# swift-nav/albatross

Measured on AMD Instinct MI355X. Metric: GP fits/sec (Gram+Chol+solve) at N=16384 fp64, higher is better.
Workload: dtype f64

## Files before the change

### albatross_amd/csrc/api.hip

```cpp
#include <algorithm>
#include <atomic>
#include <cmath>
#include <cstring>
#include <chrono>
#include <cstdio>
#include <new>
#include <thread>

#include "api_internal.h"
#include <deque>
#include <mutex>
#include <tuple>
#include <unordered_map>
#include "trace.h"
#include "pub.h"

namespace agp {

void DeviceFeatures::release() {
  for (void *&p : owned) {
    if (p) (void)hipFree(p);
    p = nullptr;
  }
  v = FeatView{};
// ... 136 lines not shown
  return n;
}

static constexpr long long BACKSUB_COOP_MAX_N = 2047;
static agp_context::Tuning read_tuning() {
  agp_context::Tuning t;
  auto flag = [](const char *name, bool dflt) {
    const char *e = getenv(name);
    return e && e[0] ? e[0] == '1' : dflt;
  };
  auto number = [](const char *name, long long dflt) {
    const char *e = getenv(name);
    return e && e[0] ? atoll(e) : dflt;
  };
  t.panel_fused = flag("AGP_PANEL_FUSED", true);
  t.step_below = number("AGP_STEP_BELOW", 4608);
  t.gram_sop = flag("AGP_GRAM_SOP", true);
  t.backsub_coop = flag("AGP_BACKSUB_COOP", true);
  t.backsub_coop_max = number("AGP_BACKSUB_COOP_MAX", BACKSUB_COOP_MAX_N);
  t.mixed_bf16 = flag("AGP_MIXED_BF16", true);
  t.mixed_f16 = flag("AGP_MIXED_F16", true);
  set_f16x2_kernel((int)number("AGP_F16X2_LDS_PAD", 8192), (int)number("AGP_F16X2_TERMS", 4), (int)number("AGP_F16X2_CHUNK", 32));
  t.mixed_nbo = number("AGP_MIXED_NBO", 512);
  t.fp64_nbo = number("AGP_FP64_NBO", 0);
  if (t.fp64_nbo <= 512 || t.fp64_nbo % 128 != 0) t.fp64_nbo = 0;
  set_bf16x3_kernel((int)number("AGP_BF16X3_KERNEL", 2), (int)number("AGP_BF16X3_LDS_PAD", 8192));
  t.sparse_pivoted = flag("AGP_SPARSE_PIVOTED", false);
  t.predict_chunk = number("AGP_PREDICT_CHUNK", 0);
  t.shard_block = number("AGP_SHARD_BLOCK", 0);
  t.shard_force_comm = flag("AGP_SHARD_FORCE_COMM", false);
  t.shard_host_pacing = flag("AGP_SHARD_HOST_PACING", false);
  if (const char *e = getenv("AGP_SHARD_MASK_GFLOP")) t.shard_mask_gflop = atof(e);
  t.merge_above = number("AGP_MERGE_ABOVE", 8704);
  return t;
}

int agp_context_create(int device_id, agp_context **out) {
  if (!out) return AGP_ERR_INVALID_ARGUMENT;
  *out = nullptr;
  int n = 0;
  if (hipGetDeviceCount(&n) != hipSuccess || n <= 0) return AGP_ERR_NO_DEVICE;
  if (device_id < 0 || device_id >= n) return AGP_ERR_INVALID_ARGUMENT;
  agp_context_impl *ctx = new (std::nothrow) agp_context_impl();
  if (!ctx) return AGP_ERR_INVALID_ARGUMENT;
  ctx->device = device_id;
  ctx->tune = read_tuning();
  agp::g_gram_sop = ctx->tune.gram_sop;
  AGP_HIP_CHECK(ctx, hipSetDevice(device_id));
  {
    int lo = 0, hi = 0;
    AGP_HIP_CHECK(ctx, hipDeviceGetStreamPriorityRange(&lo, &hi));
    AGP_HIP_CHECK(ctx, hipStreamCreateWithPriority(&ctx->stream, hipStreamNonBlocking, hi));
    AGP_HIP_CHECK(ctx, hipStreamCreateWithPriority(&ctx->stream2, hipStreamNonBlocking, lo));
    AGP_HIP_CHECK(ctx, hipStreamCreateWithPriority(&ctx->stream3, hipStreamNonBlocking, lo));
    AGP_HIP_CHECK(ctx, hipEventCreateWithFlags(&ctx->ev_inv, hipEventDisableTiming));
    AGP_HIP_CHECK(ctx, hipEventCreateWithFlags(&ctx->ev_c, hipEventDisableTiming));
    int cus = 256;
    (void)hipDeviceGetAttribute(&cus, hipDeviceAttributeMultiprocessorCount, device_id);
    ctx->cus = cus;
    const int keep = cus / 8 * 7 / 8 * 8;
    if (keep > 0 && keep < cus) {
      uint32_t mask[16] = {0};
      for (int i = 0; i < keep && i < 512; ++i) mask[i / 32] |= 1u << (i % 32);
      if (hipExtStreamCreateWithCUMask(&ctx->stream_masked, (uint32_t)((cus + 31) / 32), mask) != hipSuccess) {
        (void)hipGetLastError();
        ctx->stream_masked = nullptr;
// ... 11 lines not shown
  for (auto &e : ctx->stage_ev) AGP_HIP_CHECK(ctx, hipEventCreate(&e));
  for (auto &sl : ctx->ext.slots) AGP_HIP_CHECK(ctx, hipMalloc(&sl.dev, sizeof(DevProgram)));
  *out = ctx;
  return AGP_OK;
}

void agp_context_destroy(agp_context *c) {
  if (!c) return;
  agp_context_impl *ctx = static_cast<agp_context_impl *>(c);
  (void)hipSetDevice(ctx->device);
  (void)hipDeviceSynchronize();
  for (agp_context *h : ctx->helpers) agp_context_destroy(h);
  ctx->helpers.clear();
  for (auto &sl : ctx->ext.slots)
    if (sl.dev) (void)hipFree(sl.dev);
  for (auto e : ctx->gemm_events) (void)hipEventDestroy(e);
  for (auto e : ctx->stage_ev)
    if (e) (void)hipEventDestroy(e);
  if (ctx->partial_ws) (void)hipFree(ctx->partial_ws);
  if (ctx->ws_A) (void)agp::dev_release(ctx->ws_A);
  if (ctx->pool_A) (void)agp::dev_release(ctx->pool_A);
  if (ctx->pool_K) (void)agp::dev_release(ctx->pool_K);
  if (ctx->ws_refine) (void)hipFree(ctx->ws_refine);
  if (ctx->p32) (void)hipFree(ctx->p32);
  if (ctx->f16_scales) (void)hipFree(ctx->f16_scales);
  if (ctx->pool_L32) (void)hipFree(ctx->pool_L32);
  if (ctx->pool_aux) (void)agp::dev_release(ctx->pool_aux);
  if (ctx->pool_shard) (void)agp::dev_release(ctx->pool_shard);
  if (ctx->pool_sparse) (void)agp::dev_release(ctx->pool_sparse);
  if (ctx->pool_batch) (void)agp::dev_release(ctx->pool_batch);
  if (ctx->ws_aux) (void)hipFree(ctx->ws_aux);
  if (ctx->d_zpub) (void)hipFree(ctx->d_zpub);
  if (ctx->d_dpub) (void)hipFree(ctx->d_dpub);
  if (ctx->shard_flags) (void)hipFree(ctx->shard_flags);
  if (ctx->d_headcnt) (void)hipFree(ctx->d_headcnt);
  if (ctx->h_stage) (void)hipHostFree(ctx->h_stage);
  if (ctx->d_flags) (void)hipFree(ctx->d_flags);
  if (ctx->h_flags) (void)hipHostFree(ctx->h_flags);
  if (ctx->ev_a) (void)hipEventDestroy(ctx->ev_a);
  if (ctx->ev_b) (void)hipEventDestroy(ctx->ev_b);
  if (ctx->stream) (void)hipStreamDestroy(ctx->stream);
  if (ctx->stream2) (void)hipStreamDestroy(ctx->stream2);
  if (ctx->stream3) (void)hipStreamDestroy(ctx->stream3);
  if (ctx->ev_inv) (void)hipEventDestroy(ctx->ev_inv);
  if (ctx->stream_masked) (void)hipStreamDestroy(ctx->stream_masked);
  if (ctx->stream_comm) (void)hipStreamDestroy(ctx->stream_comm);
  if (ctx->ev_c) (void)hipEventDestroy(ctx->ev_c);
  delete ctx;
  agp::dev_cache_trim();
}

int agp_context_synchronize(agp_context *ctx) {
  if (!ctx) return AGP_ERR_INVALID_ARGUMENT;
  AGP_HIP_CHECK(ctx, hipSetDevice(ctx->device));
  AGP_HIP_CHECK(ctx, hipDeviceSynchronize());
  return AGP_OK;
}

int agp_device_malloc(agp_context *ctx, int64_t bytes, void **out) {
  if (!ctx || !out || bytes <= 0) return AGP_ERR_INVALID_ARGUMENT;
  *out = nullptr;
  AGP_HIP_CHECK(ctx, hipSetDevice(ctx->device));
  AGP_HIP_CHECK(ctx, hipMalloc(out, (size_t)bytes));
  return AGP_OK;
}

// ... 1643 lines not shown
```

### albatross_amd/csrc/chol.hip

```cpp
#include <cstdlib>
#include "common.h"
#include "mfma_f64.h"
#include "gemm_tiles.h"
#include "trsm_kernel.h"
#include "pub.h"

namespace agp {
void launch_set_identity_batched(hipStream_t s, double *B, long long ld, long long stride, long long m, long long count);

__device__ __forceinline__ double readlane_f64(double v, int lane) {
  const long long b = __double_as_longlong(v);
  const int lo = __builtin_amdgcn_readlane((int)(b & 0xffffffffll), lane);
  const int hi = __builtin_amdgcn_readlane((int)(b >> 32), lane);
  return __longlong_as_double(((long long)hi << 32) | (unsigned int)lo);
}

__device__ __forceinline__ double rsqrt_nr(double x) {
  double y = __builtin_amdgcn_rsq(x);
  const double h = 0.5 * x;
  y = y * (1.5 - h * y * y);
  y = y * (1.5 - h * y * y);
  return y;
}

struct PotrfArgs {
  double *A;
  long long lda;
  long long k0;
  int nbk;
  double *img;
  double *y;
  int *flags;
  double *scalars;
  long long batch_A = 0, batch_img = 0, batch_y = 0, batch_scalars = 0, batch_flags = 0, batch_zpub = 0;
  double *zpub = nullptr;
  long long below = 0;
  double *dpub = nullptr;
  unsigned trail_first = 0xffffffffu;
  unsigned hold_index = 0xffffffffu, hold_count = 0;
  unsigned long long *rowcnt = nullptr;
  unsigned long long rowcnt_expect = 0;
  long long trail_tiles = 0, trail_workers = 1;
};


template <int J>
__device__ __forceinline__ double bcast_row(double v) {
  double r;
  asm("s_nop 1\n\tv_mov_b64_dpp %0, %1 row_newbcast:%2 row_mask:0xf bank_mask:0xf" : "=v"(r) : "v"(v), "n"(J));
  return r;
}

template <int J>
__device__ __forceinline__ void fnmac_bcast_row(double &acc, double src, double a) {
  asm("s_nop 1\n\tv_fmac_f64_dpp %0, -%1, %2 row_newbcast:%3 row_mask:0xf bank_mask:0xf"
      : "+v"(acc) : "v"(src), "v"(a), "n"(J));
}

__device__ __forceinline__ double vmul(double a, double b) {
  double r;
  asm volatile("v_mul_f64 %0, %1, %2" : "=v"(r) : "v"(a), "v"(b));
  return r;
}
__device__ __forceinline__ double vfma(double a, double b, double c) {
  double r;
  asm volatile("v_fma_f64 %0, %1, %2, %3" : "=v"(r) : "v"(a), "v"(b), "v"(c));
  return r;
}
__device__ __forceinline__ double vfnma(double a, double b, double c) {
  double r;
  asm volatile("v_fma_f64 %0, -%1, %2, %3" : "=v"(r) : "v"(a), "v"(b), "v"(c));
  return r;
}
__device__ __forceinline__ double vrsq(double a) {
  double r;
// ... 168 lines not shown
  double *Adiag = p.A + p.k0 * p.lda + p.k0;
  if constexpr (UPD) {
    double v[NTILE];
    unsigned long long t0 = 0;
    for (int spin = 0;; ++spin) {
      bool ok = true;
#pragma unroll
      for (int t = 0; t < NTILE; ++t) v[t] = load_pub(p.dpub + t * (MB * MB) + tid);
#pragma unroll
      for (int t = 0; t < NTILE; ++t) ok = ok && !is_unpublished(v[t]);
      if (__all(ok)) break;
      if (spin == 0) t0 = __builtin_amdgcn_s_memrealtime();
      else if ((spin & 63) == 0 && poll_expired(t0, p.flags)) break;
      __builtin_amdgcn_s_sleep(2);
    }
#pragma unroll
    for (int t = 0; t < NTILE; ++t) T[t * (MB * MB) + tid] = v[t];
  } else {
    const int r = tid & 15, c = tid >> 4;
    double v[NTILE];
#pragma unroll
    for (int ib = 0; ib < NMB; ++ib)
#pragma unroll
      for (int kb = 0; kb <= ib; ++kb) {
        const int gr = ib * MB + r, gc = kb * MB + c;
        double x;
        if (gr < nbk && gc < nbk) x = (gr >= gc) ? Adiag[gc * p.lda + gr] : 0.;
        else x = (gr == gc) ? 1. : 0.;
        v[ib * (ib + 1) / 2 + kb] = x;
      }
#pragma unroll
    for (int t = 0; t < NTILE; ++t) T[t * (MB * MB) + c * MB + r] = v[t];
  }
  if (tid < NB) ys[tid] = (p.y && tid < nbk) ? p.y[tid] : 0.;
  __syncthreads();

  int bad_pivot = 0;
  if (wave == 0) micro_potrf_inv<PUB>(T + tile_off(0, 0), Wc, p.img + tile_off(0, 0), lane, ln, 0, bad_pivot);
  __syncthreads();
  AGP_PROBE(1);

#pragma unroll 1
  for (int jb = 0; jb < NMB; ++jb) {
    const int o = jb * MB;
    const double *W = Wc + (jb & 1) * (MB * MB);
    for (int ib = jb + 1 + wave; ib < NMB; ib += 4) {
      double *X = T + tile_off(ib, jb);
      v4d acc0 = v4zero(), acc1 = v4zero();
      acc0 = mfma16(W[(0 + lg) * MB + ln], X[(0 + lg) * MB + ln], acc0);
      acc1 = mfma16(W[(4 + lg) * MB + ln], X[(4 + lg) * MB + ln], acc1);
      acc0 = mfma16(W[(8 + lg) * MB + ln], X[(8 + lg) * MB + ln], acc0);
      acc1 = mfma16(W[(12 + lg) * MB + ln], X[(12 + lg) * MB + ln], acc1);
#pragma unroll
      for (int r = 0; r < 4; ++r) {
        const double x = acc0[r] + acc1[r];
        X[(lg + 4 * r) * MB + ln] = x;
        if constexpr (PUB) store_pub(p.img + tile_off(ib, jb) + (lg + 4 * r) * MB + ln, -x);
        else p.img[tile_off(ib, jb) + (lg + 4 * r) * MB + ln] = -x;
      }
    }
    if (wave == 3) {
      double zz = 0.;
#pragma unroll
      for (int c = 0; c < MB; ++c) zz += W[c * MB + ln] * ys[o + c];
      if (lane < MB) ys[o + ln] = zz;
    }
    __syncthreads();
// ... 137 lines not shown
  const double *Xd = p.A + (p.k0 - NB) * p.lda + p.k0;
  const double *Dd = p.A + p.k0 * p.lda + p.k0;
  const int ra = kb * MB + ln, rb = ib * MB + ln;
  const bool oka = ra < p.nbk, okb = rb < p.nbk;
  v4d acc[4] = {v4zero(), v4zero(), v4zero(), v4zero()};
#pragma unroll
  for (int r = 0; r < 4; ++r) {
    const int gr = ib * MB + ln, gc = kb * MB + lg + 4 * r;
    double x;
    if (gr < p.nbk && gc < p.nbk) x = (gr >= gc) ? Dd[gc * p.lda + gr] : 0.;
    else x = (gr == gc) ? 1. : 0.;
    acc[0][r] = x;
  }
  {
    double av[32], bv[32];
#pragma unroll
    for (int s2 = 0; s2 < 32; ++s2) {
      const long long k = 4 * s2 + lg;
      av[s2] = oka ? Xd[k * p.lda + ra] : 0.;
      bv[s2] = okb ? Xd[k * p.lda + rb] : 0.;
    }
#pragma unroll
    for (int s2 = 0; s2 < 32; ++s2) acc[s2 & 3] = mfma16(-av[s2], bv[s2], acc[s2 & 3]);
  }
  const v4d out = (acc[0] + acc[1]) + (acc[2] + acc[3]);
#pragma unroll
  for (int r = 0; r < 4; ++r) {
    const int gr = ib * MB + ln, gc = kb * MB + lg + 4 * r;
    store_pub(p.dpub + tile * (MB * MB) + (lg + 4 * r) * MB + ln, (gr >= gc) ? out[r] : 0.);
  }
}

template <bool UPD>
__device__ __forceinline__ void trsm_fused_body(const PotrfArgs &p, int first_block) {
  const int tid = threadIdx.x, lane = tid & 63, wave = tid >> 6;
  const int ln = lane & 15, lg = lane >> 4;
  const long long n0 = ((long long)(blockIdx.x - first_block) * 4 + wave) * 16;
  const bool active = n0 < p.below;
  const bool nok = active && n0 + ln < p.below;
  double *base = p.A + p.k0 * p.lda + (p.k0 + p.nbk) + (n0 + ln);
  const bool handed = UPD && p.rowcnt != nullptr;
  if (handed) {
    if (tid == 0) {
      const unsigned long long *c = p.rowcnt + (blockIdx.x - first_block);
      const unsigned long long t0 = __builtin_amdgcn_s_memrealtime();
      for (int spin = 1; __hip_atomic_load(c, __ATOMIC_RELAXED, __HIP_MEMORY_SCOPE_AGENT) < p.rowcnt_expect; ++spin) {
        if ((spin & 63) == 0 && poll_expired(t0, p.flags)) break;
        __builtin_amdgcn_s_sleep(8);
      }
      __atomic_thread_fence(__ATOMIC_ACQUIRE);
    }
    __syncthreads();
  }
  if (!active) return;
  v4d Y[NMB];
#pragma unroll
  for (int jb = 0; jb < NMB; ++jb)
#pragma unroll
    for (int r = 0; r < 4; ++r) {
      const int m = jb * MB + lg + 4 * r;
      Y[jb][r] = (nok && m < p.nbk) ? (handed ? load_pub(base + m * p.lda) : base[m * p.lda]) : 0.;
    }
  trsm_fused_step<0>(p, lane, Y, base, nok, lg);
  if (p.y) {
    double z[NMB][4];
    unsigned long long t0 = 0;
    for (int spin = 0;; ++spin) {
      bool ok = true;
#pragma unroll
      for (int jb = 0; jb < NMB; ++jb)
#pragma unroll
        for (int r = 0; r < 4; ++r) {
          const int m = jb * MB + lg + 4 * r;
          z[jb][r] = (m < p.nbk) ? load_pub(p.zpub + m) : 0.;
        }
#pragma unroll
      for (int jb = 0; jb < NMB; ++jb)
#pragma unroll
        for (int r = 0; r < 4; ++r) ok = ok && !is_unpublished(z[jb][r]);
      if (__all(ok)) break;
      if (spin == 0) t0 = __builtin_amdgcn_s_memrealtime();
      else if ((spin & 63) == 0 && poll_expired(t0, p.flags)) break;
      __builtin_amdgcn_s_sleep(2);
    }
    double part = 0.;
#pragma unroll
    for (int jb = 0; jb < NMB; ++jb)
#pragma unroll
      for (int r = 0; r < 4; ++r) part += Y[jb][r] * z[jb][r];
    part += __shfl_xor(part, 16, 64);
    part += __shfl_xor(part, 32, 64);
    if (lg == 0 && nok) p.y[p.nbk + n0 + ln] -= part;
  }
}

constexpr int UPD_BLOCKS = NTILE / 4;

constexpr int TRP = ST;
__device__ __forceinline__ int trail_col(int krow, int col) { return col ^ ((krow & 1) << 4); }

__device__ __forceinline__ void trail_load_pass(const double *__restrict__ P, long long ld, long long row0, long long nrows,
                                                int k0, bool vec_ok, double (&r)[16]) {
  const int t = threadIdx.x, kk = t >> 4, seg = (t & 15) * 2;
  const long long row = row0 + seg;
#pragma unroll
  for (int c = 0; c < 4; ++c) {
    const double *q = P + row + (long long)(k0 + 16 * c + kk) * ld;
    if (vec_ok && row0 + ST <= nrows) {
      const double2 a = *reinterpret_cast<const double2 *>(q);
      const double2 b = *reinterpret_cast<const double2 *>(q + 32);
      r[4 * c] = a.x; r[4 * c + 1] = a.y; r[4 * c + 2] = b.x; r[4 * c + 3] = b.y;
    } else {
#pragma unroll
      for (int e = 0; e < 4; ++e) {
        const int off = 32 * (e >> 1) + (e & 1);
        r[4 * c + e] = (row + off < nrows) ? q[off] : 0.;
      }
    }
  }
}

template <bool NEGATE>
__device__ __forceinline__ void trail_store_pass(double *__restrict__ Ls, const double (&r)[16]) {
  const int t = threadIdx.x, kk = t >> 4, seg = (t & 15) * 2;
#pragma unroll
// ... 110 lines not shown

template <bool UPD>
__global__ __launch_bounds__(256, 2) void panel_fused_kernel(PotrfArgs p) {
  __shared__ double T[POTRF_LDS_DOUBLES];
  static_assert(POTRF_LDS_DOUBLES >= 2 * 64 * TRP, "the trailing-update workgroups stage their operands in T");
  if (!UPD && blockIdx.y > 0) {
    const long long b = blockIdx.y;
    p.A += b * p.batch_A;
    p.img += b * p.batch_img;
    if (p.y) p.y += b * p.batch_y;
    if (p.zpub) p.zpub += b * p.batch_zpub;
    if (p.scalars) p.scalars += b * p.batch_scalars;
    if (p.flags) p.flags += b * p.batch_flags;
  }
  if (UPD && blockIdx.x >= p.trail_first) {
    if (blockIdx.x >= p.hold_index && blockIdx.x < p.hold_index + p.hold_count) {
      const double *last = p.img + tile_off(NMB - 1, NMB - 1) + MB * MB - 1;
      const unsigned long long t0 = __builtin_amdgcn_s_memrealtime();
      for (int spin = 1; is_unpublished(load_pub(last)); ++spin) {
        if ((spin & 63) == 0 && poll_expired(t0, p.flags)) break;
        __builtin_amdgcn_s_sleep(64);
      }
      return;
    }
    trail_update_body(p, (long long)(blockIdx.x - p.trail_first) - (blockIdx.x > p.hold_index ? (long long)p.hold_count : 0), T);
    return;
  }
  __builtin_amdgcn_s_setprio(AGP_CHAIN_PRIO);
  if (blockIdx.x == 0) {
    potrf_diag_body<true, UPD>(p, T);
  } else if (UPD && blockIdx.x <= UPD_BLOCKS) {
    diag_update_body(p, (int)(blockIdx.x - 1) * 4 + (int)(threadIdx.x >> 6));
  } else {
    trsm_fused_body<UPD>(p, UPD ? 1 + UPD_BLOCKS : 1);
  }
}


static void launch_potrf(hipStream_t s, double *A, long long lda, long long k0, int nbk, double *img,
                         double *y, int *flags, double *scalars) {
  PotrfArgs p;
  p.A = A; p.lda = lda; p.k0 = k0; p.nbk = nbk;
  p.img = img + (k0 / NB) * (long long)IMG_DOUBLES;
  p.y = y ? y + k0 : nullptr;
  p.flags = flags; p.scalars = scalars;
  hipLaunchKernelGGL(potrf_diag_kernel, dim3(1), dim3(256), 0, s, p);
}

static void timed_gemm(hipStream_t s, FactorTimers *timers, double *C, long long lda, const double *P,
                       const double *Q, long long M, long long N, long long K, bool bulk, int variant = -1,
                       const float *P32 = nullptr, long long ld32 = 0) {
  if (!bulk) {
    launch_gemm_nt_sub(s, C, lda, P, lda, false, Q, lda, false, M, N, K, true);
    return;
  }
  BulkTiming bt;
  const bool timed = timers && timers->ev && timers->used + 2 <= timers->n_ev;
  if (timed) { bt.e0 = timers->ev[timers->used]; bt.e1 = timers->ev[timers->used + 1]; }
  if (variant >= 0) launch_trailing_update_as(variant, s, C, lda, P, Q, lda, M, K, timed ? &bt : nullptr, P32, P32, ld32);
  else launch_trailing_update(s, C, lda, P, Q, lda, M, K, timed ? &bt : nullptr);
  if (timed && bt.flops > 0.) {
    timers->flops[timers->used / 2] = bt.flops;
    timers->used += 2;
  }
}

constexpr long long FUSED_BELOW = 4608;
// ... 71 lines not shown
  const long long b0 = k_begin / NB, b1 = (k_end + NB - 1) / NB;
  if (want_step && ctx->tune.step_below > 0 && ctx->dpub_cap < b1) {
    (void)hipStreamSynchronize(ctx->stream);
    if (ctx->d_dpub) (void)hipFree(ctx->d_dpub);
    ctx->d_dpub = nullptr;
    ctx->d_rowcnt = nullptr;
    ctx->dpub_cap = 0;
    const long long cap = (b1 + 31) / 32 * 32;
    if (hipMalloc(&ctx->d_dpub, sizeof(double) * (size_t)cap * (IMG_DOUBLES + 2)) == hipSuccess) {
      ctx->dpub_cap = cap;
      ctx->d_rowcnt = reinterpret_cast<unsigned long long *>(ctx->d_dpub + cap * (long long)IMG_DOUBLES);
    }
    else (void)hipGetLastError();
  }
  const long long cnt_img = (b1 - b0) * (long long)IMG_DOUBLES, cnt_z = k_end - k_begin;
  if (ctx->d_dpub && ctx->dpub_cap >= b1) {
    prep->fill(ctx->d_rowcnt + 2 * b0, 0ull, 2 * (b1 - b0));
    prep->sentinel(ctx->d_dpub + b0 * (long long)IMG_DOUBLES, cnt_img);
  }
  prep->sentinel(invd + b0 * (long long)IMG_DOUBLES, cnt_img);
  prep->sentinel(ctx->d_zpub + k_begin, cnt_z);
  if (want_step && k_begin == 0 && ctx->d_headcnt && ctx->tune.merge_above > 0 && k_end > ctx->tune.merge_above && !prep->full()) {
    prep->fill(ctx->d_headcnt, 0ull, agp_context::HEADCNT_WORDS);
    ctx->headcnt_ready = true;
  }
  ctx->zpub_ready_n = k_end;
  ctx->img_ready = invd;
  return true;
}

void panel_fused_prepare(agp_context *ctx, hipStream_t s, double *invd, long long k_begin, long long k_end, bool want_step) {
  PrepArgs prep;
  if (panel_fused_plan(ctx, invd, k_begin, k_end, want_step, &prep)) launch_prep(s, prep);
}

static void panel_phase(agp_context *ctx, hipStream_t s, double *A, long long n, long long lda, double *invd,
                        double *y, long long K0, long long kend, FactorTimers *timers, bool step_mode = false,
                        long long mark_after = -1, hipEvent_t mark_event = nullptr) {
  if (kend != n) step_mode = false;
  const bool inner_left = !step_mode && (n - K0) > INNER_LEFT_ABOVE;
  const bool fused = ctx->tune.panel_fused && ctx->d_zpub && ctx->zpub_ready_n >= kend && ctx->img_ready == invd &&
                     ((n - K0) <= FUSED_BELOW || step_mode);
  for (long long k = K0; k < kend; k += NB) {
    const int nbk = (int)((n - k < NB) ? n - k : NB);
    if (mark_event && k == mark_after + NB) (void)hipEventRecord(mark_event, s);
    if (inner_left && k > K0) {
      const double *P = A + K0 * lda + k;
      timed_gemm(s, timers, A + k * lda + k, lda, P, P, n - k, nbk, k - K0, false);
    }
    const long long below = n - (k + nbk);
    if (fused) {
      PotrfArgs pa;
      pa.A = A; pa.lda = lda; pa.k0 = k; pa.nbk = nbk;
      pa.img = invd + (k / NB) * (long long)IMG_DOUBLES;
      pa.y = y ? y + k : nullptr;
      pa.flags = ctx->d_flags; pa.scalars = ctx->d_scalars;
      pa.zpub = y ? ctx->d_zpub + k : nullptr;
      pa.below = below > 0 ? below : 0;
      if (step_mode && k > K0) {
        pa.dpub = ctx->d_dpub + (k / NB) * (long long)IMG_DOUBLES;
        unsigned grid = (unsigned)(1 + UPD_BLOCKS + (pa.below + 63) / 64);
        if (pa.below > 0) {
          const long long nt = (pa.below + 63) / 64;
          pa.trail_first = grid;
          pa.rowcnt = ctx->d_rowcnt + (k + NB) / 64;
          pa.rowcnt_expect = 2ull * (unsigned long long)((k - K0) / NB);
          const long long tiles = nt * (nt + 1) / 2 + 2 * nt;
          const long long slots = step_slots(ctx), first_round = ctx->cus, ncrit = grid;
          long long workers = tiles, nhold = 0;
          if (ncrit + workers > first_round && ncrit < first_round) {
            nhold = tiles <= 1200 ? ncrit : 1 + UPD_BLOCKS;
            const long long cap = slots - ncrit - nhold;
            if (workers > cap) workers = cap;
            if (ncrit + workers <= first_round) nhold = 0;
          } else if (workers > slots - ncrit) {
            workers = slots - ncrit;
          }
          if (workers < 2 * nt) workers = 2 * nt < tiles ? 2 * nt : tiles;
          pa.trail_tiles = tiles;
          pa.trail_workers = workers;
          grid += (unsigned)workers;
          if (nhold > 0) {
            pa.hold_index = (unsigned)first_round;
            pa.hold_count = (unsigned)nhold;
            grid += (unsigned)nhold;
          }
        }
        hipLaunchKernelGGL(panel_fused_kernel<true>, dim3(grid), dim3(256), 0, s, pa);
        ++ctx->sched.panels_step;
      } else {
        hipLaunchKernelGGL(panel_fused_kernel<false>, dim3((unsigned)(1 + (pa.below + 63) / 64)), dim3(256), 0, s, pa);
// ... 407 lines not shown
```

### albatross_amd/csrc/common.h

```cpp
#pragma once
#include <hip/hip_runtime.h>
#include <cstdint>
#include <cstdio>
#include <string>
#include <utility>
#include <vector>

#include "../../include/albatross_amd.h"
#include "cov_eval.h"

#define AGP_CHAIN_PRIO 3

namespace agp {

constexpr int NB = 128;
constexpr int NBO = 512;
constexpr int MB = 16;
constexpr int NMB = NB / MB;

struct FeatView {
  const double *coords;
  const long long *ids;
  const double *scales;
  long long n;
// ... 58 lines not shown
  size_t pool_aux_bytes = 0;
  int update_variant = -1;
  long long nbo_override = 0;
  long long nbo_wide = 0;
  double *pool_shard = nullptr;
  size_t pool_shard_bytes = 0;
  double *pool_sparse = nullptr;
  size_t pool_sparse_bytes = 0;
  double *pool_batch = nullptr;
  size_t pool_batch_bytes = 0;
  double *d_zpub = nullptr;
  long long zpub_cap = 0, zpub_ready_n = 0;
  double *d_dpub = nullptr;
  long long dpub_cap = 0;
  int cus = 256;
  long long step_slots = 0;
  struct Tuning {
    bool panel_fused = true;
    long long step_below = 4608;
    bool gram_sop = true;
    long long fp64_nbo = 0;
    long long mixed_nbo = 512;
    bool mixed_f16 = true;
    bool mixed_bf16 = true;
    long long backsub_coop_max = 2047;
    bool backsub_coop = true;
    bool sparse_pivoted = false;
    long long predict_chunk = 0;
    long long shard_block = 0;
    bool shard_force_comm = false;
    bool shard_host_pacing = false;
    double shard_mask_gflop = 40.;
    long long merge_above = 8704;
  } tune;
  unsigned long long *d_rowcnt = nullptr;
  void *h_stage = nullptr;
  size_t h_stage_bytes = 0;
  static constexpr long long HEADCNT_WORDS = 256;
  unsigned long long *d_headcnt = nullptr;
  bool headcnt_ready = false;
  struct ScheduleRecord {
    static constexpr unsigned MERGED = 1, STEP = 2, THROTTLED = 4, MASKED = 8, SINGLE = 16;
    enum Backsub { BS_NONE = 0, BS_COOP_DIRECT = 1, BS_COOP_FLAGS = 2, BS_WIDE = 3, BS_CHAIN = 4 };
    static constexpr unsigned INV_EARLY = 1, INV_LAST_STEP = 2, INV_TAIL = 4;
    long long n = 0;
    long long steps = 0, steps_dropped = 0;
    long long kend[HEADCNT_WORDS] = {};
    unsigned bits[HEADCNT_WORDS] = {};
    long long panels_step = 0, panels_fused = 0, panels_split = 0;
    int backsub = BS_NONE;
    long long bs_done = 0;
    unsigned inv_bits = 0;
    int handover_timeout = 0;
    long long demotions = 0;
    void reset_factor(long long n_) {
      n = n_;
      steps = steps_dropped = 0;
      panels_step = panels_fused = panels_split = 0;
      inv_bits = 0;
      handover_timeout = 0;
    }
    void add_step(long long end, unsigned b) {
      if (steps < HEADCNT_WORDS) { kend[steps] = end; bits[steps] = b; ++steps; }
      else ++steps_dropped;
    }
  } sched;
  double *bs_W = nullptr;
  long long bs_BW = 0, bs_done = 0;
  hipEvent_t ev_inv = nullptr;
  const double *img_ready = nullptr;
  bool prep_external = false;
  hipStream_t stream_comm = nullptr;
  unsigned long long *shard_flags = nullptr;
  unsigned long long shard_seq[16] = {};
  unsigned long long shard_probe_seq = 0;
  int shard_host_pacing = -1;
  bool shard_probe_ok = false;
};

struct agp_fit_slab {
  double *base = nullptr;
  size_t bytes = 0;
  int refs = 0;
};

struct agp_fit {
  agp_context *ctx = nullptr;
  agp_fit_slab *slab = nullptr;
  size_t A_bytes = 0;
  int device = 0;
  int64_t n = 0;
// ... 153 lines not shown
```

### albatross_amd/csrc/debug_api.hip

```cpp
#include <algorithm>
#include <cstdio>
#include "common.h"
#include "api_internal.h"
#include "mfma_f64.h"
#include "shard_internal.h"
#include <cstdlib>
#include <cstring>
#include <new>

#define AGP_DEBUG_API __attribute__((visibility("default")))

namespace agp {

__global__ void mfma_tile_kernel(const double *A, const double *B, double *D) {
  const int l = threadIdx.x;
  v4d acc = v4zero();
  acc = mfma16(A[(l & 15) * 4 + (l >> 4)], B[(l >> 4) * 16 + (l & 15)], acc);
  for (int r = 0; r < 4; ++r) D[((l >> 4) + 4 * r) * 16 + (l & 15)] = acc[r];
}

template <int NACC>
__global__ __launch_bounds__(256) void mfma_clock_kernel(unsigned long long *out, int iters, double a0, double b0) {
  v4d acc[NACC];
#pragma unroll
// ... 806 lines not shown
  }
  AGP_HIP_CHECK(ctx, hipMemsetAsync(ctx->d_flags, 0, 4 * sizeof(int), ctx->stream));
  AGP_HIP_CHECK(ctx, hipMemsetAsync(ctx->d_scalars, 0, 4 * sizeof(double), ctx->stream));
  factor_lower(ctx, dA, n, lda, dI, dy, nullptr);
  AGP_HIP_CHECK(ctx, hipStreamSynchronize(ctx->stream));
  AGP_HIP_CHECK(ctx, hipGetLastError());
  AGP_HIP_CHECK(ctx, hipMemcpy(A, dA, ab, hipMemcpyDeviceToHost));
  if (y) AGP_HIP_CHECK(ctx, hipMemcpy(y, dy, sizeof(double) * (size_t)n, hipMemcpyDeviceToHost));
  int flags[4];
  double scal[4];
  AGP_HIP_CHECK(ctx, hipMemcpy(flags, ctx->d_flags, sizeof(flags), hipMemcpyDeviceToHost));
  AGP_HIP_CHECK(ctx, hipMemcpy(scal, ctx->d_scalars, sizeof(scal), hipMemcpyDeviceToHost));
  if (log_det) *log_det = 2. * scal[0];
  if (bad_pivot) *bad_pivot = flags[1] ? flags[1] - 1 : -1;
  (void)hipFree(dA); (void)hipFree(dI);
  if (dy) (void)hipFree(dy);
  ctx->sched.backsub = agp_context::ScheduleRecord::BS_NONE;
  ctx->sched.bs_done = 0;
  ctx->sched.handover_timeout = flags[2];
  return AGP_OK;
}

constexpr int64_t SCHED_HEADER = 20;
AGP_DEBUG_API int agp_debug_schedule(agp_context *ctx, int64_t *out, int64_t cap) {
  if (!ctx || !out || cap < 0) return AGP_ERR_INVALID_ARGUMENT;
  const agp_context::ScheduleRecord &r = ctx->sched;
  int64_t w[SCHED_HEADER + 2 * agp_context::HEADCNT_WORDS] = {};
  w[0] = r.n; w[1] = r.steps; w[2] = r.steps_dropped;
  w[3] = r.panels_step; w[4] = r.panels_fused; w[5] = r.panels_split;
  w[6] = r.backsub; w[7] = r.bs_done; w[8] = r.inv_bits; w[9] = r.handover_timeout; w[10] = r.demotions;
  w[11] = ctx->step_slots; w[12] = ctx->cus; w[13] = ctx->stream_masked ? 1 : 0;
  w[14] = ctx->tune.step_below; w[15] = ctx->tune.panel_fused ? 1 : 0; w[16] = ctx->tune.merge_above;
  w[17] = ctx->tune.backsub_coop ? 1 : 0; w[18] = ctx->tune.fp64_nbo;
  for (long long i = 0; i < r.steps; ++i) {
    w[SCHED_HEADER + 2 * i] = r.kend[i];
    w[SCHED_HEADER + 2 * i + 1] = r.bits[i];
  }
  const int64_t total = SCHED_HEADER + 2 * agp_context::HEADCNT_WORDS;
  for (int64_t i = 0; i < cap && i < total; ++i) out[i] = w[i];
  return AGP_OK;
}

}

namespace agp {
__global__ __launch_bounds__(256) void mfma_peak_kernel(double *sink, int iters, double a0, double b0) {
  v4d acc[8];
#pragma unroll
  for (int i = 0; i < 8; ++i) acc[i] = v4zero();
  double a = a0 + threadIdx.x * 1e-9, b = b0 - threadIdx.x * 1e-9;
  for (int it = 0; it < iters; ++it) {
#pragma unroll
    for (int i = 0; i < 8; ++i) acc[i] = mfma16(a, b, acc[i]);
  }
  double s = 0.;
#pragma unroll
  for (int i = 0; i < 8; ++i) s += acc[i][0] + acc[i][1] + acc[i][2] + acc[i][3];
  if (s == 123.456) sink[0] = s;
}

static int mfma_f64_peak(hipStream_t s, int iters, double *tflops) {
  double *sink = nullptr;
  if (hipMalloc(&sink, 8) != hipSuccess) return AGP_ERR_HIP;
  hipEvent_t e0, e1;
  (void)hipEventCreate(&e0);
  (void)hipEventCreate(&e1);
// ... 70 lines not shown
```

Baseline: 34.69.

## Run Cholesky tail panels in one persistent kernel with dataflow task scheduling

Replaces the per-panel step-mode launches for the Cholesky tail with a persistent resident kernel. Block 0 factors the diagonal blocks, and worker blocks pull tasks (diag update, row update, TRSM solve, trailing tiles) from an atomic ticket counter. They wait on per-tile version and solved flags, so dependent work across consecutive panels can overlap without kernel boundaries. This aims to remove launch and barrier overhead in the small tail steps. It adds spin-wait synchronisation complexity, extra flag buffers, and a risk of stalls or contention if the task ordering is poor.

Result: slower. 32.88, median of 2 (-5.2%).

```diff
diff --git a/albatross_amd/csrc/api.hip b/albatross_amd/csrc/api.hip
--- a/albatross_amd/csrc/api.hip
+++ b/albatross_amd/csrc/api.hip
@@ -192,6 +192,7 @@
   t.shard_host_pacing = flag("AGP_SHARD_HOST_PACING", false);
   if (const char *e = getenv("AGP_SHARD_MASK_GFLOP")) t.shard_mask_gflop = atof(e);
   t.merge_above = number("AGP_MERGE_ABOVE", 8704);
+  t.tail_resident = flag("AGP_TAIL_RESIDENT", true);
   return t;
 }
 
@@ -269,6 +270,7 @@
   if (ctx->ws_aux) (void)hipFree(ctx->ws_aux);
   if (ctx->d_zpub) (void)hipFree(ctx->d_zpub);
   if (ctx->d_dpub) (void)hipFree(ctx->d_dpub);
+  if (ctx->d_res) (void)hipFree(ctx->d_res);
   if (ctx->shard_flags) (void)hipFree(ctx->shard_flags);
   if (ctx->d_headcnt) (void)hipFree(ctx->d_headcnt);
   if (ctx->h_stage) (void)hipHostFree(ctx->h_stage);
diff --git a/albatross_amd/csrc/chol.hip b/albatross_amd/csrc/chol.hip
--- a/albatross_amd/csrc/chol.hip
+++ b/albatross_amd/csrc/chol.hip
@@ -41,6 +41,7 @@
   unsigned long long *rowcnt = nullptr;
   unsigned long long rowcnt_expect = 0;
   long long trail_tiles = 0, trail_workers = 1;
+  bool y_pub = false;
 };
 
 
@@ -275,7 +276,7 @@
 #pragma unroll
     for (int t = 0; t < NTILE; ++t) T[t * (MB * MB) + c * MB + r] = v[t];
   }
-  if (tid < NB) ys[tid] = (p.y && tid < nbk) ? p.y[tid] : 0.;
+  if (tid < NB) ys[tid] = (p.y && tid < nbk) ? (p.y_pub ? load_pub(p.y + tid) : p.y[tid]) : 0.;
   __syncthreads();
 
   int bad_pivot = 0;
@@ -479,17 +480,17 @@
 }
 
 template <bool UPD>
-__device__ __forceinline__ void trsm_fused_body(const PotrfArgs &p, int first_block) {
+__device__ __forceinline__ void trsm_fused_body(const PotrfArgs &p, long long rb) {
   const int tid = threadIdx.x, lane = tid & 63, wave = tid >> 6;
   const int ln = lane & 15, lg = lane >> 4;
-  const long long n0 = ((long long)(blockIdx.x - first_block) * 4 + wave) * 16;
+  const long long n0 = (rb * 4 + wave) * 16;
   const bool active = n0 < p.below;
   const bool nok = active && n0 + ln < p.below;
   double *base = p.A + p.k0 * p.lda + (p.k0 + p.nbk) + (n0 + ln);
   const bool handed = UPD && p.rowcnt != nullptr;
   if (handed) {
     if (tid == 0) {
-      const unsigned long long *c = p.rowcnt + (blockIdx.x - first_block);
+      const unsigned long long *c = p.rowcnt + rb;
       const unsigned long long t0 = __builtin_amdgcn_s_memrealtime();
       for (int spin = 1; __hip_atomic_load(c, __ATOMIC_RELAXED, __HIP_MEMORY_SCOPE_AGENT) < p.rowcnt_expect; ++spin) {
         if ((spin & 63) == 0 && poll_expired(t0, p.flags)) break;
@@ -537,7 +538,11 @@
       for (int r = 0; r < 4; ++r) part += Y[jb][r] * z[jb][r];
     part += __shfl_xor(part, 16, 64);
     part += __shfl_xor(part, 32, 64);
-    if (lg == 0 && nok) p.y[p.nbk + n0 + ln] -= part;
+    if (lg == 0 && nok) {
+      double *yr = p.y + p.nbk + n0 + ln;
+      if (p.y_pub) store_pub(yr, load_pub(yr) - part);
+      else *yr -= part;
+    }
   }
 }
 
@@ -714,7 +719,191 @@
   } else if (UPD && blockIdx.x <= UPD_BLOCKS) {
     diag_update_body(p, (int)(blockIdx.x - 1) * 4 + (int)(threadIdx.x >> 6));
   } else {
-    trsm_fused_body<UPD>(p, UPD ? 1 + UPD_BLOCKS : 1);
+    trsm_fused_body<UPD>(p, (long long)blockIdx.x - (UPD ? 1 + UPD_BLOCKS : 1));
+  }
+}
+
+struct ResidentGeom {
+  long long n = 0, K0 = 0;
+  int jb = 1, je = 1;
+  enum Kind { T_UPD, T_ROW, T_SOLVE, T_TRAIL, T_END };
+  __host__ __device__ long long below(int j) const {
+    const long long b = n - (K0 + (long long)NB * j) - NB;
+    return b > 0 ? b : 0;
+  }
+  __host__ __device__ long long nrb(int j) const { return (below(j) + ST - 1) / ST; }
+  __host__ __device__ long long near(int j) const { const long long t = nrb(j); return t >= 2 ? 2 * t - 1 : t; }
+  __host__ __device__ long long far(int j) const { const long long t = nrb(j); return t * (t + 1) / 2 - near(j); }
+  __host__ __device__ Kind task(long long t, int &j, long long &idx) const {
+    for (j = jb; j < je; ++j) {
+      const long long nr = nrb(j);
+      if (t < UPD_BLOCKS) { idx = t; return T_UPD; }
+      t -= UPD_BLOCKS;
+      if (t < 2 * nr) { idx = t; return T_ROW; }
+      t -= 2 * nr;
+      if (t < nr) { idx = t; return T_SOLVE; }
+      t -= nr;
+      if (j > jb) {
+        const long long f = far(j - 1);
+        if (t < f) { --j; idx = near(j) + t; return T_TRAIL; }
+        t -= f;
+      }
+      const long long ne = near(j);
+      if (t < ne) { idx = t; return T_TRAIL; }
+      t -= ne;
+    }
+    j = je - 1;
+    if (t < far(j)) { idx = near(j) + t; return T_TRAIL; }
+    return T_END;
+  }
+  long long count() const {
+    long long c = far(je - 1);
+    for (int j = jb; j < je; ++j) c += UPD_BLOCKS + 3 * nrb(j) + near(j) + (j > jb ? far(j - 1) : 0);
+    return c;
+  }
+};
+
+struct ResidentArgs {
+  ResidentGeom g;
+  double *A;
+  long long lda;
+  double *img, *dpub, *zpub, *y;
+  int *flags;
+  double *scalars;
+  unsigned long long *rowcnt;
+  unsigned long long *ver;
+  unsigned long long *solved;
+  unsigned long long *ticket;
+  unsigned long long tag, ticket0;
+  long long ntasks;
+  unsigned hold_index;
+};
+
+__device__ __forceinline__ PotrfArgs resident_panel(const ResidentArgs &r, int j) {
+  PotrfArgs p;
+  const long long k = r.g.K0 + (long long)NB * j;
+  p.A = r.A; p.lda = r.lda; p.k0 = k;
+  p.nbk = (int)((r.g.n - k < NB) ? r.g.n - k : NB);
+  p.img = r.img + (k / NB) * (long long)IMG_DOUBLES;
+  p.y = r.y ? r.y + k : nullptr;
+  p.flags = r.flags; p.scalars = r.scalars;
+  p.zpub = r.y ? r.zpub + k : nullptr;
+  p.below = r.g.below(j);
+  p.dpub = r.dpub + (k / NB) * (long long)IMG_DOUBLES;
+  p.rowcnt = r.rowcnt + (k + NB) / ST;
+  p.rowcnt_expect = 2ull * (unsigned long long)j;
+  p.y_pub = true;
+  return p;
+}
+
+__device__ __forceinline__ long long res_tile(long long gi, long long gj) { return gi * (gi + 1) / 2 + gj; }
+
+__device__ __forceinline__ void res_wait(const unsigned long long *c, unsigned long long target, int *flags) {
+  if (__hip_atomic_load(c, __ATOMIC_RELAXED, __HIP_MEMORY_SCOPE_AGENT) >= target) return;
+  const unsigned long long t0 = __builtin_amdgcn_s_memrealtime();
+  for (int spin = 1; __hip_atomic_load(c, __ATOMIC_RELAXED, __HIP_MEMORY_SCOPE_AGENT) < target; ++spin) {
+    if ((spin & 63) == 0 && (poll_expired(t0, flags) || __hip_atomic_load(flags + 2, __ATOMIC_RELAXED, __HIP_MEMORY_SCOPE_AGENT))) break;
+    __builtin_amdgcn_s_sleep(4);
+  }
+}
+
+__device__ __forceinline__ void res_publish(unsigned long long *c, unsigned long long value) {
+  __builtin_amdgcn_s_waitcnt(0);
+  __syncthreads();
+  if (threadIdx.x == 0) __hip_atomic_store(c, value, __ATOMIC_RELEASE, __HIP_MEMORY_SCOPE_AGENT);
+}
+
+__device__ __forceinline__ void res_wait_update(const ResidentArgs &r, int j, long long gi, long long gj) {
+  if (j - 1 < r.g.jb) return;
+  if (threadIdx.x == 0) {
+    const unsigned long long need = r.tag | (unsigned long long)(j - 1);
+    res_wait(r.solved + gi, need, r.flags);
+    if (gj != gi) res_wait(r.solved + gj, need, r.flags);
+    res_wait(r.ver + res_tile(gi, gj), need, r.flags);
+    __builtin_amdgcn_fence(__ATOMIC_ACQUIRE, "agent");
+  }
+  __syncthreads();
+}
+
+__global__ __launch_bounds__(256, 2) void tail_resident_kernel(ResidentArgs r) {
+  __shared__ double T[POTRF_LDS_DOUBLES];
+  __shared__ long long s_task;
+  static_assert(POTRF_LDS_DOUBLES >= 2 * 64 * TRP, "the update tasks stage their operands in T");
+  const int tid = threadIdx.x;
+  if (blockIdx.x == 0) {
+    __builtin_amdgcn_s_setprio(AGP_CHAIN_PRIO);
+    for (int j = r.g.jb; j < r.g.je; ++j) {
+      PotrfArgs p = resident_panel(r, j);
+      if (j > r.g.jb) __syncthreads();
+      potrf_diag_body<true, true>(p, T);
+    }
+    return;
+  }
+  if (blockIdx.x == r.hold_index) {
+    const PotrfArgs p = resident_panel(r, r.g.je - 1);
+    const double *last = p.img + tile_off(NMB - 1, NMB - 1) + MB * MB - 1;
+    const unsigned long long t0 = __builtin_amdgcn_s_memrealtime();
+    for (int spin = 1; is_unpublished(load_pub(last)); ++spin) {
+      if ((spin & 63) == 0 && poll_expired(t0, r.flags)) break;
+      __builtin_amdgcn_s_sleep(64);
+    }
+    return;
+  }
+  for (;;) {
+    if (tid == 0) s_task = (long long)(__hip_atomic_fetch_add(r.ticket, 1ull, __ATOMIC_RELAXED, __HIP_MEMORY_SCOPE_AGENT) - r.ticket0);
+    __syncthreads();
+    const long long t = s_task;
+    __syncthreads();
+    if (t < 0) return;
+    int j = 0;
+    long long idx = 0;
+    const ResidentGeom::Kind kind = t < r.ntasks ? r.g.task(t, j, idx) : ResidentGeom::T_END;
+    if (kind == ResidentGeom::T_END) return;
+    const PotrfArgs p = resident_panel(r, j);
+    const long long g0 = 2ll * j;
+    if (kind == ResidentGeom::T_UPD) {
+      __builtin_amdgcn_s_setprio(AGP_CHAIN_PRIO);
+      if (j - 1 >= r.g.jb) {
+        if (tid == 0) {
+          const unsigned long long need = r.tag | (unsigned long long)(j - 1);
+          const bool two = p.nbk > ST;
+          res_wait(r.solved + g0, need, r.flags);
+          if (two) res_wait(r.solved + g0 + 1, need, r.flags);
+          res_wait(r.ver + res_tile(g0, g0), need, r.flags);
+          if (two) {
+            res_wait(r.ver + res_tile(g0 + 1, g0), need, r.flags);
+            res_wait(r.ver + res_tile(g0 + 1, g0 + 1), need, r.flags);
+          }
+          __builtin_amdgcn_fence(__ATOMIC_ACQUIRE, "agent");
+        }
+        __syncthreads();
+      }
+      diag_update_body(p, (int)idx * 4 + (tid >> 6));
+    } else if (kind == ResidentGeom::T_ROW) {
+      __builtin_amdgcn_s_setprio(0);
+      const long long nr = r.g.nrb(j), bj = idx / nr, bi = idx % nr;
+      res_wait_update(r, j, g0 + 2 + bi, g0 + bj);
+      trail_tile64<true>(p.A + p.k0 * p.lda + p.k0, p.A + (p.k0 - NB) * p.lda + p.k0, p.lda, p.below + NB, (2 + bi) * ST, bj * ST,
+                         T, p.rowcnt + bi);
+    } else if (kind == ResidentGeom::T_SOLVE) {
+      __builtin_amdgcn_s_setprio(AGP_CHAIN_PRIO);
+      trsm_fused_body<true>(p, idx);
+      res_publish(r.solved + g0 + 2 + idx, r.tag | (unsigned long long)j);
+    } else {
+      __builtin_amdgcn_s_setprio(0);
+      const int ntr = (int)r.g.nrb(j);
+      long long id = idx;
+      int bj = 0;
+      while (id >= ntr - bj) {
+        id -= ntr - bj;
+        ++bj;
+      }
+      const long long bi = bj + id, gi = g0 + 2 + bi, gj = g0 + 2 + bj;
+      res_wait_update(r, j, gi, gj);
+      const long long t0 = p.k0 + NB;
+      trail_tile64(p.A + t0 * p.lda + t0, p.A + (p.k0 - NB) * p.lda + t0, p.lda, p.below, bi * ST, (long long)bj * ST, T);
+      res_publish(r.ver + res_tile(gi, gj), r.tag | (unsigned long long)j);
+    }
   }
 }
 
@@ -852,6 +1041,69 @@
 void panel_fused_prepare(agp_context *ctx, hipStream_t s, double *invd, long long k_begin, long long k_end, bool want_step) {
   PrepArgs prep;
   if (panel_fused_plan(ctx, invd, k_begin, k_end, want_step, &prep)) launch_prep(s, prep);
+}
+
+static long long resident_slots(agp_context *ctx) {
+  if (ctx->res_slots <= 0) {
+    int per_cu = 0;
+    if (hipOccupancyMaxActiveBlocksPerMultiprocessor(&per_cu, tail_resident_kernel, 256, 0) != hipSuccess || per_cu <= 0) {
+      (void)hipGetLastError();
+      per_cu = 1;
+    }
+    ctx->res_slots = (long long)per_cu * ctx->cus;
+  }
+  return ctx->res_slots;
+}
+
+static bool resident_buffers(agp_context *ctx, hipStream_t s, long long rows) {
+  const long long t = (rows + ST - 1) / ST, words = t * (t + 1) / 2 + t + 1;
+  if (ctx->res_cap < words) {
+    (void)hipStreamSynchronize(ctx->stream);
+    if (ctx->d_res) (void)hipFree(ctx->d_res);
+    ctx->d_res = nullptr;
+    ctx->res_cap = 0;
+    const long long cap = (words + 4095) / 4096 * 4096;
+    if (hipMalloc(&ctx->d_res, sizeof(unsigned long long) * (size_t)cap) != hipSuccess) { (void)hipGetLastError(); return false; }
+    if (hipMemsetAsync(ctx->d_res, 0, sizeof(unsigned long long) * (size_t)cap, s) != hipSuccess) {
+      (void)hipGetLastError();
+      (void)hipFree(ctx->d_res);
+      ctx->d_res = nullptr;
+      return false;
+    }
+    ctx->res_cap = cap;
+    ctx->res_epoch = 0;
+    ctx->res_ticket = 0;
+  }
+  return true;
+}
+
+static void launch_tail_resident(agp_context *ctx, hipStream_t s, double *A, long long n, long long lda, double *invd, double *y,
+                                 long long K0, int jb, int je) {
+  ResidentArgs r;
+  r.g.n = n; r.g.K0 = K0; r.g.jb = jb; r.g.je = je;
+  r.A = A; r.lda = lda;
+  r.img = invd; r.dpub = ctx->d_dpub; r.zpub = ctx->d_zpub; r.y = y;
+  r.flags = ctx->d_flags; r.scalars = ctx->d_scalars;
+  r.rowcnt = ctx->d_rowcnt;
+  const long long t = (n - K0 + ST - 1) / ST;
+  r.ticket = ctx->d_res;
+  r.ver = ctx->d_res + 1;
+  r.solved = r.ver + t * (t + 1) / 2;
+  r.tag = (++ctx->res_epoch) << 32;
+  r.ticket0 = ctx->res_ticket;
+  r.ntasks = r.g.count();
+  long long workers = resident_slots(ctx) - 2;
+  if (workers > r.ntasks) workers = r.ntasks;
+  if (workers < 1) workers = 1;
+  long long grid = 1 + workers;
+  r.hold_index = 0xffffffffu;
+  if (grid >= ctx->cus) {
+    r.hold_index = (unsigned)ctx->cus;
+    ++grid;
+  }
+  hipLaunchKernelGGL(tail_resident_kernel, dim3((unsigned)grid), dim3(256), 0, s, r);
+  if (hipPeekAtLastError() == hipSuccess) ctx->res_ticket += (unsigned long long)(r.ntasks + workers);
+  else ctx->res_cap = 0;
 }
 
 static void panel_phase(agp_context *ctx, hipStream_t s, double *A, long long n, long long lda, double *invd,
@@ -877,6 +1129,20 @@
       pa.flags = ctx->d_flags; pa.scalars = ctx->d_scalars;
       pa.zpub = y ? ctx->d_zpub + k : nullptr;
       pa.below = below > 0 ? below : 0;
+      if (step_mode && k > K0 && ctx->tune.tail_resident && resident_buffers(ctx, s, n - K0)) {
+        const int P = (int)((n - K0 + NB - 1) / NB), j0 = (int)((k - K0) / NB);
+        const long long m = mark_event ? (mark_after + NB - K0) / NB : -1;
+        if (m > j0 && m < P) {
+          launch_tail_resident(ctx, s, A, n, lda, invd, y, K0, j0, (int)m);
+          (void)hipEventRecord(mark_event, s);
+          launch_tail_resident(ctx, s, A, n, lda, invd, y, K0, (int)m, P);
+        } else {
+          launch_tail_resident(ctx, s, A, n, lda, invd, y, K0, j0, P);
+        }
+        ctx->sched.panels_step += P - j0;
+        ctx->sched.panels_resident += P - j0;
+        break;
+      }
       if (step_mode && k > K0) {
         pa.dpub = ctx->d_dpub + (k / NB) * (long long)IMG_DOUBLES;
         unsigned grid = (unsigned)(1 + UPD_BLOCKS + (pa.below + 63) / 64);
diff --git a/albatross_amd/csrc/common.h b/albatross_amd/csrc/common.h
--- a/albatross_amd/csrc/common.h
+++ b/albatross_amd/csrc/common.h
@@ -114,7 +114,12 @@
     bool shard_host_pacing = false;
     double shard_mask_gflop = 40.;
     long long merge_above = 8704;
+    bool tail_resident = true;
   } tune;
+  unsigned long long *d_res = nullptr;
+  long long res_cap = 0;
+  unsigned long long res_epoch = 0, res_ticket = 0;
+  long long res_slots = 0;
   unsigned long long *d_rowcnt = nullptr;
   void *h_stage = nullptr;
   size_t h_stage_bytes = 0;
@@ -130,6 +135,7 @@
     long long kend[HEADCNT_WORDS] = {};
     unsigned bits[HEADCNT_WORDS] = {};
     long long panels_step = 0, panels_fused = 0, panels_split = 0;
+    long long panels_resident = 0;
     int backsub = BS_NONE;
     long long bs_done = 0;
     unsigned inv_bits = 0;
@@ -138,7 +144,7 @@
     void reset_factor(long long n_) {
       n = n_;
       steps = steps_dropped = 0;
-      panels_step = panels_fused = panels_split = 0;
+      panels_step = panels_fused = panels_split = panels_resident = 0;
       inv_bits = 0;
       handover_timeout = 0;
     }
diff --git a/albatross_amd/csrc/debug_api.hip b/albatross_amd/csrc/debug_api.hip
--- a/albatross_amd/csrc/debug_api.hip
+++ b/albatross_amd/csrc/debug_api.hip
@@ -862,6 +862,7 @@
   w[11] = ctx->step_slots; w[12] = ctx->cus; w[13] = ctx->stream_masked ? 1 : 0;
   w[14] = ctx->tune.step_below; w[15] = ctx->tune.panel_fused ? 1 : 0; w[16] = ctx->tune.merge_above;
   w[17] = ctx->tune.backsub_coop ? 1 : 0; w[18] = ctx->tune.fp64_nbo;
+  w[19] = r.panels_resident;
   for (long long i = 0; i < r.steps; ++i) {
     w[SCHED_HEADER + 2 * i] = r.kend[i];
     w[SCHED_HEADER + 2 * i + 1] = r.bits[i];
```
